# joaospinto/sip_optimal_control

Hardware: AMD Instinct MI355X
Metric: Riccati sweeps/sec (backward+forward) (higher is better)
Workload: dtype f64

## Files before the change

### sip_optimal_control_amd/csrc/chain_qw16.hpp

```cpp
#pragma once
#include <hip/hip_runtime.h>
#include <type_traits>

#include "dpp_blocks_gen.hpp"

namespace sipamd {

template <int I, int E, class F>
__device__ __forceinline__ void sfor(F &&f) {
  if constexpr (I < E) {
    f(std::integral_constant<int, I>{});
    sfor<I + 1, E>(f);
  }
}
template <int I, int E, class F>
__device__ __forceinline__ void sfor_down(F &&f) {
  if constexpr (I > E) {
    f(std::integral_constant<int, I>{});
    sfor_down<I - 1, E>(f);
  }
}

template <int K>
__device__ __forceinline__ double bcast(double x) {
  double und;
  asm volatile("" : "=v"(und));
  return __builtin_amdgcn_update_dpp(und, x, 0x150 + K, 0xf, 0xf, false);
}

__device__ __forceinline__ double rsqrt_nr(double d) {
  const double y = __builtin_amdgcn_rsq(d);
  const double s = d * y;
  const double e = __builtin_fma(-s, y, 1.0);
  const double t = __builtin_fma(0.375, e, 0.5);
  return __builtin_fma(y * e, t, y);
}

__device__ __forceinline__ double rcp_nr(double d) {
  const double y = __builtin_amdgcn_rcp(d);
  const double e = __builtin_fma(-d, y, 1.0);
  const double t = __builtin_fma(e, e, e);
  return __builtin_fma(y, t, y);
}

template <int S>
__device__ __forceinline__ bool chol_ldl_dpp(double (&A)[S], double (&dinv)[S],
                                             const int c) {
#ifdef SIP_QW16_CHOL_SELECT
  unsigned long long failmask = 0;
  sfor<0, S>([&](auto kk) {
    constexpr int k = decltype(kk)::value;
    const double d = bcast<k>(A[k]);
    failmask |= __ballot(d <= 0.0);
    const double y2 = rcp_nr(d);
    dinv[k] = y2;
    const double upd = (c > k && c < S) ? A[k] * y2 : 0.0;
    rank1<S - k - 1, k, true, false>(A + k + 1, A + k + 1, upd);
  });
  return ((failmask >> (__lane_id() & 63)) & 1ull) != 0;
#else
  double dmin = __builtin_inf();
  sfor<0, S>([&](auto kk) {
    constexpr int k = decltype(kk)::value;
    const double d = bcast<k>(A[k]);
    asm("v_min_f64 %0, %1, %2" : "=v"(dmin) : "v"(dmin), "v"(d));
    const double own = A[k] * ((c > k && c < S) ? 1.0 : 0.0);
    const double y2 = rcp_nr(d);
    dinv[k] = y2;
    const double upd = own * y2;
    rank1<S - k - 1, k, true, false>(A + k + 1, A + k + 1, upd);
  });
  return dmin <= 0.0;
#endif
}

template <int S>
__device__ __forceinline__ void ldl_solve_dpp(const double (&Lt)[S],
                                              const double (&dinv)[S],
                                              double (&X)[S]) {
  sfor<0, S>([&](auto jj) {
    constexpr int j = decltype(jj)::value;
    X[j] *= dinv[j];
    rank1<S - j - 1, j, true, (j == 0)>(X + j + 1, Lt + j + 1, X[j]);
  });
  double acc[S];
  sfor<0, S>([&](auto jj) { acc[decltype(jj)::value] = 0.0; });
  sfor_down<S - 1, -1>([&](auto jj) {
    constexpr int j = decltype(jj)::value;
    X[j] = __builtin_fma(-dinv[j], acc[j], X[j]);
    spread<j, false, false>(acc, Lt[j], X[j]);
  });
}

template <int N, int M, bool SYM = false>
struct ChainLayout {
  static constexpr int QLEN = SYM ? N * (N + 1) / 2 : N * N;
  static constexpr int RLEN = SYM ? M * (M + 1) / 2 : M * M;
  static constexpr int NODE = QLEN + N;
  static constexpr int EDGE = N * N + 2 * N * M + RLEN;
  static constexpr int VNODE = 2 * N;
  static constexpr int VEDGE = M;
  static constexpr int GAIN = M * N + M;
  static constexpr int WSN = N * N + 2 * N;
};

template <int N, bool EXPORT = false>
__device__ __forceinline__ bool node_factor(const double (&V)[N], const double dl,
                                            const int c, const double (&E)[N],
                                            const double (&tv)[N], double (&W)[N],
                                            double (&X)[N], double *Lt = nullptr) {
  const double sdi = rsqrt_nr(dl);
  const double sd = dl * sdi;
  double S[N], A[N], rinv[N];
  sfor<0, N>([&](auto ii) { S[decltype(ii)::value] = 0.0; });
  spread<N, false, true>(S, sd, sd);
  sfor<0, N>([&](auto ii) {
    constexpr int r = decltype(ii)::value;
    A[r] = __builtin_fma(S[r], V[r], E[r]);
  });
  const bool fail = chol_ldl_dpp<N>(A, rinv, c);
  if constexpr (EXPORT)
    sfor<0, N>([&](auto ii) { Lt[decltype(ii)::value] = A[decltype(ii)::value]; });
  sfor<0, N>([&](auto ii) { X[decltype(ii)::value] = E[decltype(ii)::value]; });
  spreadv<N, false>(X, sdi, tv);
  ldl_solve_dpp<N>(A, rinv, X);
  sfor<0, N>([&](auto ii) { S[decltype(ii)::value] = 0.0; });
  spread<N, false, true>(S, sdi, sdi);
  sfor<0, N>([&](auto ii) {
    constexpr int r = decltype(ii)::value;
    W[r] = (E[r] - X[r]) * S[r];
  });
  return fail;
}

#ifndef SIP_LQR_NT_SOL
#define SIP_LQR_NT_SOL 0
#endif
#ifndef SIP_LQR_NT_IN
#define SIP_LQR_NT_IN 2
#endif
#ifndef SIP_LQR_NT_FAB
#define SIP_LQR_NT_FAB SIP_LQR_NT_IN
#endif
#ifndef SIP_LQR_NT_FSP
#define SIP_LQR_NT_FSP 0
#endif
typedef __attribute__((address_space(3))) char lds_char;
typedef const __attribute__((address_space(3))) double lds_cdouble;

#ifdef SIP_LQR_STAMPS
#define SIP_STAMP(var)                                                         \
  do {                                                                         \
    __builtin_amdgcn_sched_barrier(0);                                         \
    asm volatile("s_memtime %0\n\ts_waitcnt lgkmcnt(0)" : "=s"(var)::"memory"); \
    __builtin_amdgcn_sched_barrier(0);                                         \
  } while (0)
#define SIP_STAMP_ARG , unsigned long long *__restrict__ stamps
#define SIP_SEG(k)                                                             \
  do {                                                                         \
    unsigned long long now_;                                                   \
    SIP_STAMP(now_);                                                           \
    seg[k] += now_ - seg_last;                                                 \
    seg_last = now_;                                                           \
  } while (0)
#else
#define SIP_SEG(k)                                                             \
  do {                                                                         \
  } while (0)
#define SIP_STAMP(var)                                                         \
  do {                                                                         \
  } while (0)
#define SIP_STAMP_ARG
#endif

template <int PIECES>
struct StageDma {
  static constexpr int INSTR = (4 * PIECES + 63) / 64;
  static constexpr int BYTES = INSTR * 1024;
  static constexpr int ROW_BYTES = PIECES * 16;
#ifdef SIP_QW16_DMA_PLAIN
  static constexpr int GROUP = 1;
#else
  static constexpr int GROUP = 4;
#endif
  static constexpr unsigned BIAS = (GROUP - 1) * 1024u;
  unsigned off[INSTR > 0 ? INSTR : 1];
  __device__ __forceinline__ void init(const int lane,
                                       const unsigned problem_stride_bytes,
                                       const unsigned max_rel) {
    sfor<0, INSTR>([&](auto jj) {
      constexpr int j = decltype(jj)::value;
      const unsigned q = (unsigned)(j * 64 + lane) < 4u * PIECES ? (unsigned)(j * 64 + lane) : 4u * PIECES - 1u;
      unsigned rr = q / PIECES;
      const unsigned within = q - rr * PIECES;
      rr = rr < max_rel ? rr : max_rel;
      off[j] = rr * problem_stride_bytes + within * 16u + BIAS - (unsigned)(j % GROUP) * 1024u;
    });
  }
  template <int AUX = 0>
  __device__ __forceinline__ void issue(const char *base, lds_char *dst,
                                        const int lane) const {
    const char *lowered = base - BIAS;
    sfor<0, INSTR>([&](auto jj) {
      constexpr int j = decltype(jj)::value;
      __builtin_amdgcn_global_load_lds((const __attribute__((address_space(1))) void *)(lowered + off[j]),
                                       (__attribute__((address_space(3))) void *)(dst + (j - j % GROUP) * 1024), 16,
                                       (j % GROUP) * 1024, AUX);
    });
  }
};

template <int DWORDS>
struct StageDmaDwords {
  static constexpr int INSTR = (4 * DWORDS + 63) / 64;
  static constexpr int BYTES = (INSTR * 256 + 1023) / 1024 * 1024;
  static constexpr int ROW_BYTES = DWORDS * 4;
  unsigned off[INSTR > 0 ? INSTR : 1];
  __device__ __forceinline__ void init(const int lane, const unsigned problem_stride_bytes, const unsigned max_rel) {
    sfor<0, INSTR>([&](auto jj) {
      constexpr int j = decltype(jj)::value;
      const unsigned q = (unsigned)(j * 64 + lane) < 4u * DWORDS ? (unsigned)(j * 64 + lane) : 4u * DWORDS - 1u;
      unsigned rr = q / DWORDS;
      const unsigned within = q - rr * DWORDS;
      rr = rr < max_rel ? rr : max_rel;
      off[j] = rr * problem_stride_bytes + within * 4u;
    });
  }
  template <int AUX = 0>
  __device__ __forceinline__ void issue(const char *base, lds_char *dst, const int lane) const {
    sfor<0, INSTR>([&](auto jj) {
      constexpr int j = decltype(jj)::value;
      __builtin_amdgcn_global_load_lds((const __attribute__((address_space(1))) void *)(base + off[j]),
                                       (__attribute__((address_space(3))) void *)(dst + j * 256), 4, 0, AUX);
    });
  }
};

template <int PIECES>
struct StageDmaRows {
  static constexpr int IP = (PIECES + 63) / 64;
  static constexpr int INSTR = 4 * IP;
  static constexpr int ROW_BYTES = IP * 1024;
  static constexpr int BYTES = 4 * ROW_BYTES;
  static constexpr bool RAGGED = PIECES % 64 != 0;
  unsigned vo_main, vo_tail;
  unsigned long long row[4];
  __device__ __forceinline__ void init(const int lane,
                                       const unsigned problem_stride_bytes,
                                       const unsigned max_rel) {
    vo_main = (unsigned)lane * 16u;
    const unsigned last = (unsigned)(PIECES - 1 - 64 * (IP - 1));
    vo_tail = ((unsigned)lane < last ? (unsigned)lane : last) * 16u;
    sfor<0, 4>([&](auto rq) {
      constexpr unsigned r = decltype(rq)::value;
      row[r] = (unsigned long long)(r < max_rel ? r : max_rel) * problem_stride_bytes;
    });
  }
  template <int AUX = 0>
  __device__ __forceinline__ void issue(const char *base, lds_char *dst,
                                        const int lane) const {
    sfor<0, 4>([&](auto rq) {
      constexpr int r = decltype(rq)::value;
      const char *region = base + row[r];
      sfor<0, IP>([&](auto jq) {
        constexpr int jj = decltype(jq)::value;
        constexpr int g = jj / 4;
        const unsigned vo = (RAGGED && jj == IP - 1) ? vo_tail : vo_main;
        __builtin_amdgcn_global_load_lds(
            (const __attribute__((address_space(1))) void *)(region + g * 4096 + vo),
            (__attribute__((address_space(3))) void *)(dst + r * ROW_BYTES + g * 4096), 16, (jj % 4) * 1024, AUX);
      });
    });
  }
};

template <int N, int M, bool WPACK, bool SPLIT = false, bool SYM = false>
struct StagedCfg {
  using L = ChainLayout<N, M, SYM>;
  static_assert(!SYM || (L::QLEN % 2 == 0 && L::RLEN % 2 == 0 && N % 2 == 0 && M % 2 == 0),
                "the symmetric-packed kernels are instantiated where every block stays a whole number of 16-byte pieces");
  static constexpr int AB = N * N + N * M;
  static constexpr int STG = L::NODE + L::EDGE - (SPLIT ? AB : 0);
  static constexpr int WSN =
      WPACK ? ((N * (N + 1) / 2 + 2 * N + 1) / 2) * 2 : L::WSN;
  using BV = StageDma<(L::VNODE + L::VEDGE + 1) / 2>;
  using BMflat = StageDma<(STG + 1) / 2>;
  using BMrows = StageDmaRows<(STG + 1) / 2>;
  struct NoStream {
    static constexpr int INSTR = 0, BYTES = 0, ROW_BYTES = 0;
  };
  static_assert(!SPLIT || AB % 2 == 0, "the split kernels are instantiated for even N (A | B in whole 16-byte pieces)");
  using BA = std::conditional_t<SPLIT, StageDmaRows<AB / 2>, NoStream>;
  static constexpr int SCR_BYTES_ = ((4 * 2 * N + N) * 8 + 1023) / 1024 * 1024;
  static constexpr int waves_per_cu(int bm_bytes) {
    const int per_wave = 2 * (bm_bytes + BA::BYTES + BV::BYTES) + SCR_BYTES_;
    const int w = 163840 / per_wave;
    return w > 4 ? 4 : w;
  }
#ifdef SIP_QW16_DMA_FLAT
  using BM = BMflat;
#else
  using BM = std::conditional_t<SPLIT || waves_per_cu(BMrows::BYTES) >= waves_per_cu(BMflat::BYTES), BMrows, BMflat>;
#endif
  static constexpr int B_BYTES = BM::BYTES + BA::BYTES + BV::BYTES;
  using FA = StageDma<(N * N + N * M + 1) / 2>;
  using FG = std::conditional_t<L::GAIN % 2 == 0, StageDma<L::GAIN / 2>, StageDmaDwords<2 * L::GAIN>>;
  using FW = StageDma<WSN / 2>;
  using FC = std::conditional_t<N % 2 == 0, StageDma<N / 2>, StageDmaDwords<2 * N>>;
  static constexpr int F_BYTES = FA::BYTES + FG::BYTES + FW::BYTES + FC::BYTES;
  static constexpr int F_GLDS = FA::INSTR + FG::INSTR + FW::INSTR + FC::INSTR;
  static constexpr int B_NBUF = 2;
  static constexpr int lds_main(int fbufs) {
    return B_NBUF * B_BYTES > fbufs * F_BYTES ? B_NBUF * B_BYTES : fbufs * F_BYTES;
  }
  static constexpr int waves_with(int fbufs) {
    const int w = 163840 / (lds_main(fbufs) + SCR_BYTES_);
    return w > 4 ? 4 : w;
  }
#ifdef SIP_LQR_FNBUF
  static constexpr int F_NBUF = SIP_LQR_FNBUF;
#else
  static constexpr int F_NBUF = (waves_with(2) > waves_with(3) || lds_main(3) + SCR_BYTES_ > 65536) ? 2 : 3;
#endif
  static constexpr int LDS_MAIN = lds_main(F_NBUF);
  static constexpr int SCR_BYTES = ((4 * 2 * N + N) * 8 + 1023) / 1024 * 1024;
  static constexpr int LDS_BYTES = LDS_MAIN + SCR_BYTES;
  static constexpr bool OK = N <= 16;
  static constexpr bool WIDE = N % 2 == 0;
};

template <int N, int M, bool STAGED, bool WPACK, bool SPLIT = false, bool SYM = false>
__global__ __launch_bounds__(64) void chain_factor_solve_qw16(
    const double *__restrict__ mats, const double *__restrict__ vecs,
    double *__restrict__ sol, double *__restrict__ gains,
    double *__restrict__ wsp, int *__restrict__ status, const long batch,
    const int T, const int mode, double *__restrict__ gfac,
    const double *__restrict__ ab, const long ab_pstride, const long ab_sstride SIP_STAMP_ARG) {
  constexpr bool VDIST = N == 16;
  static_assert(N >= 1 && N <= 16, "one problem per 16-lane row");
  static_assert(M >= 1 && M <= 16, "");
  using L = ChainLayout<N, M, SYM>;
  using C = StagedCfg<N, M, WPACK, SPLIT, SYM>;
  static_assert(!SPLIT || (STAGED && WPACK), "the split kernel is the staged one");
  static_assert(!SYM || (STAGED && !VDIST), "the symmetric-packed layout is served by the staged kernels");
  unsigned long long ts_begin = 0, ts_term = 0, ts_bwd = 0, ts_root = 0,
                     ts_end = 0, ts_a = 0, ts_b = 0, acc_bwait = 0,
                     acc_fwait = 0;
  (void)ts_begin, (void)ts_term, (void)ts_bwd, (void)ts_root, (void)ts_end,
      (void)ts_a, (void)ts_b, (void)acc_bwait, (void)acc_fwait;
  unsigned long long seg[12] = {0, 0, 0, 0, 0, 0, 0, 0, 0, 0, 0, 0}, seg_last = 0;
  (void)seg, (void)seg_last;
  SIP_STAMP(ts_begin);
  static_assert(!STAGED || C::LDS_BYTES <= 65536, "the LDS images of this shape exceed a workgroup's 64 KiB");
  constexpr int STG = C::STG;
  constexpr int OFF_M = L::NODE + (SPLIT ? 0 : N * N + N * M), OFF_R = OFF_M + N * M;
  constexpr int VSTG = L::VNODE + L::VEDGE;
  constexpr int WSN = C::WSN;
  constexpr int WG = WPACK ? N * (N + 1) / 2 : N * N;

  extern __shared__ double lds_raw[];
  lds_char *const lds = (lds_char *)lds_raw;

  const int lane = threadIdx.x & 63;
  const int c = lane & 15;
  const int rr = lane >> 4;
  const long p0 = (long)blockIdx.x * 4;
  long p = p0 + rr;
  const bool valid = p < batch;
  if (!valid)
    p = batch - 1;
  const bool isM = c < N;
  const bool isV = c == N;
  const int cm = isM ? c : N - 1;
  const int cu = c < M ? c : M - 1;

  const long mats_len = (long)(T + 1) * L::NODE + (long)T * (STG - L::NODE);
  const long vecs_len = (long)(T + 1) * L::VNODE + (long)T * L::VEDGE;
  const long gains_len = (long)T * L::GAIN;
  const long ws_len = (long)(T + 1) * WSN;
  const double *pm = mats + p * mats_len;
  const double *pv = vecs + p * vecs_len;
  double *ps = sol + p * vecs_len;
  double *pg = gains + p * gains_len;
  double *pw = wsp + p * ws_len;
  const unsigned max_rel =
      (unsigned)((batch - 1 - p0) < 3 ? (batch - 1 - p0) : 3);

  double E[N];
  sfor<0, N>([&](auto ii) {
    constexpr int r = decltype(ii)::value;
    E[r] = (c == r) ? 1.0 : 0.0;
  });

  auto spill_row_offsets = [&](int(&woff)[N]) {
    sfor<0, N>([&](auto kk) {
      constexpr int k = decltype(kk)::value;
      if constexpr (WPACK) {
        const int lo = k < cm ? k : cm, hi = k < cm ? cm : k;
        woff[k] = lo * N - (lo * (lo - 1)) / 2 + (hi - lo);
      } else {
        woff[k] = cm * N + k;
      }
    });
  };

  int stat = 0;
  double W[N], V[N], t[N], vch[N];
  double vd = 0.0, td = 0.0, qd = 0.0;
  auto sum4 = [](const double (&a)[4]) { return (a[0] + a[1]) + (a[2] + a[3]); };

  const __amdgpu_buffer_rsrc_t ws_rsrc = __builtin_amdgcn_make_buffer_rsrc(
      (void *)(wsp + p0 * ws_len), 0, (int)((max_rel + 1) * ws_len * 8), 0x00020000);
  const int wstore_base = (valid && isM)
                              ? (int)(rr * ws_len * 8) + (c * N - (c * (c - 1)) / 2 - c) * 8
                              : 0x7ffff000;

  typedef __attribute__((address_space(3))) double lds_double;
  lds_char *const scr = lds + C::LDS_MAIN;
  lds_double *const my_t = (lds_double *)(scr + rr * (2 * N * 8));
  lds_double *const my_v = my_t + N;
  lds_cdouble *const zeros = (lds_cdouble *)(scr + 4 * (2 * N * 8));
  if constexpr (STAGED) {
    if (lane < N)
      ((lds_double *)zeros)[lane] = 0.0;
  }

  auto load_vq = [&](auto nm, auto nv, double(&Vq)[N]) {
    if constexpr (SYM) {
      const int base_c = cm * N - (cm * (cm - 1)) / 2 - cm;
      sfor<0, N>([&](auto ii) {
        constexpr int r = decltype(ii)::value;
        constexpr int base_r = r * N - (r * (r - 1)) / 2 - r;
        const int off = r >= cm ? base_c + r : base_r + cm;
        auto src = isV ? nv + r : nm + off;
        Vq[r] = *src;
      });
    } else {
    auto src = isV ? nv : nm + cm * N;
    sfor<0, N>([&](auto ii) {
      constexpr int r = decltype(ii)::value;
      Vq[r] = src[r];
    });
    }
    if constexpr (VDIST)
      qd = nv[cm];
  };

  struct NodeTail {
    double dl, cv[N], dv[N];
    double cd;
  };
  auto load_tail = [&](auto nm, auto nv, NodeTail &nt) {
    const double d = nm[L::QLEN + cm];
    nt.dl = isM ? d : 1.0;
    nt.cd = VDIST ? nv[N + cm] : 0.0;
    if constexpr (std::is_same_v<decltype(nm), lds_cdouble *>) {
      auto csrc = isV ? nv + N : zeros, dsrc = isV ? nm + L::QLEN : zeros;
      sfor<0, N>([&](auto ii) {
        constexpr int r = decltype(ii)::value;
        nt.cv[r] = csrc[r];
        nt.dv[r] = dsrc[r];
      });
    } else {
      sfor<0, N>([&](auto ii) {
        constexpr int r = decltype(ii)::value;
        nt.cv[r] = isV ? nv[N + r] : 0.0;
        nt.dv[r] = isV ? nm[L::QLEN + r] : 0.0;
      });
    }
  };
  auto finish_node = [&](const int i, const NodeTail &nt) {
    const double dl = nt.dl;
    const unsigned long long bad = __ballot(isM && dl <= 0.0);
    const bool bad_row = ((bad >> (lane & 48)) & 0xffffull) != 0;
    if (stat == 0 && bad_row)
      stat = 1;
    double tv[N], X[N];
    sfor<0, N>([&](auto ii) {
      constexpr int r = decltype(ii)::value;
      tv[r] = nt.cv[r] - nt.dv[r] * V[r];
    });
    if constexpr (STAGED && C::WIDE) {
      if (isV) {
        typedef double d2 __attribute__((ext_vector_type(2)));
        typedef __attribute__((address_space(3))) d2 lds_d2;
        lds_d2 *const t2 = (lds_d2 *)my_t, *const v2 = (lds_d2 *)my_v;
        sfor<0, N / 2>([&](auto kk) {
          constexpr int k = decltype(kk)::value;
          t2[k] = d2{tv[2 * k], tv[2 * k + 1]};
          v2[k] = d2{V[2 * k], V[2 * k + 1]};
        });
      }
    } else if constexpr (STAGED) {
      if (isV) {
        sfor<0, N>([&](auto ii) {
          constexpr int r = decltype(ii)::value;
          my_t[r] = tv[r];
          my_v[r] = V[r];
        });
      }
    } else {
      sfor<0, N>([&](auto ii) {
        constexpr int r = decltype(ii)::value;
        t[r] = tv[r];
        vch[r] = V[r];
      });
    }
    if constexpr (VDIST)
      td = nt.cd - dl * vd;
    SIP_SEG(7);
    const bool ffail = node_factor<N>(V, dl, c, E, tv, W, X);
    SIP_SEG(8);
    if (stat == 0 && ffail)
      stat = 2;
    if constexpr (VDIST) {
      const double phi = rsqrt_nr(dl) * td;
      double acc[4] = {0.0, 0.0, 0.0, 0.0};
      dotv<N, true>(acc, phi, X);
      if (valid)
        pw[(long)i * WSN + WG + N + c] = sum4(acc);
    }
    if (valid && isV) {
      double *hn = pw + (long)i * WSN + WG + N;
      sfor<0, N>([&](auto ii) { hn[decltype(ii)::value] = X[decltype(ii)::value]; });
    }
    if constexpr (WPACK) {
      sfor<0, N>([&](auto ii) {
        constexpr int r = decltype(ii)::value;
        const int vo = (r >= c) ? wstore_base : 0x7ffff000;
        typedef unsigned int u32x2 __attribute__((ext_vector_type(2)));
        __builtin_amdgcn_raw_buffer_store_b64(__builtin_bit_cast(u32x2, X[r]), ws_rsrc, vo + r * 8,
                                              i * (WSN * 8), 0);
      });
    } else if (valid && isM) {
      double *wn = pw + (long)i * WSN + c * N;
      sfor<0, N>(
          [&](auto ii) { wn[decltype(ii)::value] = X[decltype(ii)::value]; });
    }
  };

  auto backward_edge = [&](const int i, auto nm, auto ea, auto nv, NodeTail &nt) {

    double F[N], Aaug[N], Bcol[N];
    double Hc[M], G[M], rinvG[M], H[M], K[M];
    {
      auto msrc = isV ? nv + L::VNODE : nm + (OFF_M + cm);
      sfor<0, M>([&](auto jj) {
        constexpr int j = decltype(jj)::value;
        if constexpr (SYM) {
          const int lo = j < cu ? j : cu, hi = j < cu ? cu : j;
          G[j] = nm[OFF_R + lo * M - (lo * (lo - 1)) / 2 + (hi - lo)];
        } else
        G[j] = nm[OFF_R + cu * M + j];
        H[j] = isV ? msrc[j] : msrc[j * N];
      });
    }
    if constexpr (STAGED && C::WIDE) {
      typedef double d2 __attribute__((ext_vector_type(2)));
      typedef const __attribute__((address_space(3))) d2 lds_cd2;
      lds_cd2 *a_src = (lds_cd2 *)(isV ? (lds_cdouble *)my_t : ea + cm * N);
      lds_cd2 *f_src = (lds_cd2 *)(isV ? (lds_cdouble *)my_v : zeros);
      lds_cd2 *b_src = (lds_cd2 *)(ea + N * N + cu * N);
      sfor<0, N / 2>([&](auto kk) {
        constexpr int k = decltype(kk)::value;
        const d2 a2 = a_src[k], f2 = f_src[k], b2 = b_src[k];
        Aaug[2 * k] = a2[0], Aaug[2 * k + 1] = a2[1];
        F[2 * k] = f2[0], F[2 * k + 1] = f2[1];
        Bcol[2 * k] = b2[0], Bcol[2 * k + 1] = b2[1];
      });
    } else if constexpr (STAGED) {
      lds_cdouble *a_src = isV ? (lds_cdouble *)my_t : ea + cm * N;
      lds_cdouble *f_src = isV ? (lds_cdouble *)my_v : zeros;
      lds_cdouble *b_src = ea + N * N + cu * N;
      sfor<0, N>([&](auto kk) {
        constexpr int k = decltype(kk)::value;
        Aaug[k] = a_src[k], F[k] = f_src[k], Bcol[k] = b_src[k];
      });
    } else {
      sfor<0, N>([&](auto kk) {
        constexpr int k = decltype(kk)::value;
        Aaug[k] = isV ? t[k] : ea[cm * N + k];
        F[k] = isV ? vch[k] : 0.0;
        Bcol[k] = ea[N * N + cu * N + k];
      });
    }
    rank1x<N, N, true>(F, W, Aaug);
    if (valid && isV) {
      double *gn = pw + (long)(i + 1) * WSN + WG;
      sfor<0, N>(
          [&](auto ii) { gn[decltype(ii)::value] = F[decltype(ii)::value]; });
    }
    double gd = 0.0, hd = 0.0, hf[M], kf[M];
    if constexpr (VDIST) {
      double acc[4] = {0.0, 0.0, 0.0, 0.0};
      dotv<N, true>(acc, td, W);
      gd = vd + sum4(acc);
      if (valid)
        pw[(long)(i + 1) * WSN + WG + c] = gd;
    }
    SIP_SEG(2);
    asm volatile("" ::: "memory");
    double Vn[N];
    load_vq(nm, nv, Vn);

    sfor<0, M>([&](auto jj) { Hc[decltype(jj)::value] = 0.0; });
    spreadx<M, N, false>(Hc, Bcol, W);
    rank1x<M, N, true>(G, Hc, Bcol);
    SIP_SEG(3);
    const bool gfail = chol_ldl_dpp<M>(G, rinvG, c);
    if (mode == 1 && valid) {
      double *gf = gfac + (p * (long)T + i) * (M * M + M);
      if (c < M)
        sfor<0, M>([&](auto jj) { gf[c * M + decltype(jj)::value] = G[decltype(jj)::value]; });
      if (c == 0)
        sfor<0, M>([&](auto jj) { gf[M * M + decltype(jj)::value] = rinvG[decltype(jj)::value]; });
    }
    SIP_SEG(4);
    if (stat == 0 && gfail)
      stat = 3;

    spreadx<M, N, false>(H, Bcol, F);
    if constexpr (VDIST) {
      double acc[4] = {0.0, 0.0, 0.0, 0.0};
      dotv<N, true>(acc, gd, Bcol);
      hd = nv[L::VNODE + cu] + sum4(acc);
    }
    sfor<0, M>(
        [&](auto jj) { K[decltype(jj)::value] = H[decltype(jj)::value]; });
    ldl_solve_dpp<M>(G, rinvG, K);
    sfor<0, M>(
        [&](auto jj) { K[decltype(jj)::value] = -K[decltype(jj)::value]; });
    if (valid && c <= N) {
      double *gi = pg + (long)i * L::GAIN + c * M;
      sfor<0, M>(
          [&](auto jj) { gi[decltype(jj)::value] = K[decltype(jj)::value]; });
    }
    if constexpr (VDIST) {
      double Lf[M][M];
      sfor<0, M>([&](auto jj) {
        constexpr int j = decltype(jj)::value;
        hf[j] = bcast<j>(hd);
        sfor<0, j>([&](auto iv) {
          constexpr int i2 = decltype(iv)::value;
          Lf[j][i2] = bcast<i2>(G[j]);
        });
      });
      sfor<0, M>([&](auto jj) {
        constexpr int j = decltype(jj)::value;
        double w = hf[j];
        sfor<0, j>([&](auto iv) { w = __builtin_fma(-Lf[j][decltype(iv)::value], kf[decltype(iv)::value], w); });
        kf[j] = w * rinvG[j];
      });
      sfor_down<M - 1, -1>([&](auto jj) {
        constexpr int j = decltype(jj)::value;
        double a = 0.0;
        sfor<j + 1, M>([&](auto iv) { a = __builtin_fma(Lf[decltype(iv)::value][j], kf[decltype(iv)::value], a); });
        kf[j] = __builtin_fma(-rinvG[j], a, kf[j]);
      });
      sfor<0, M>([&](auto jj) { kf[decltype(jj)::value] = -kf[decltype(jj)::value]; });
      if (valid && c == 0) {
        double *gk = pg + (long)i * L::GAIN + N * M;
        sfor<0, M>([&](auto jj) { gk[decltype(jj)::value] = kf[decltype(jj)::value]; });
      }
    }

    SIP_SEG(5);
    spreadx<N, N, false>(Vn, Aaug, F);
    asm volatile("" ::: "memory");
    load_tail(nm, nv, nt);
    asm volatile("" ::: "memory");
    spreadx<N, M, true>(Vn, K, H);
    sfor<0, N>(
        [&](auto ii) { V[decltype(ii)::value] = Vn[decltype(ii)::value]; });
    if constexpr (VDIST) {
      double acc[4] = {0.0, 0.0, 0.0, 0.0};
      dotv<N, true>(acc, gd, Aaug);
      double kh = 0.0;
      sfor<0, M>([&](auto jj) { kh = __builtin_fma(K[decltype(jj)::value], hf[decltype(jj)::value], kh); });
      vd = qd + sum4(acc) + kh;
    }
    SIP_SEG(6);
    asm volatile("" ::: "memory");
  };

  if (mode != 2) {
  typename C::BM dma_bm;
  typename C::BA dma_ba;
  typename C::BV dma_bv;
  auto issue_backward = [&](const int i, lds_char *buf) {
    dma_bm.template issue<SIP_LQR_NT_IN>((const char *)(mats + p0 * mats_len + (long)i * STG), buf, lane);
    if constexpr (SPLIT)
      dma_ba.template issue<SIP_LQR_NT_IN>((const char *)(ab + p0 * ab_pstride + (long)i * ab_sstride),
                                           buf + C::BM::BYTES, lane);
    dma_bv.template issue<SIP_LQR_NT_IN>((const char *)(vecs + p0 * vecs_len + (long)i * VSTG),
                                         buf + C::BM::BYTES + C::BA::BYTES, lane);
  };
  if constexpr (STAGED) {
    dma_bm.init(lane, (unsigned)(mats_len * 8), max_rel);
    if constexpr (SPLIT)
      dma_ba.init(lane, (unsigned)(ab_pstride * 8), max_rel);
    dma_bv.init(lane, (unsigned)(vecs_len * 8), max_rel);
    if (T > 0)
      issue_backward(T - 1, lds + ((T - 1) & 1) * C::B_BYTES);
  }
  {
    NodeTail nt;
    load_vq(pm + (long)T * STG, pv + (long)T * VSTG, V);
    if constexpr (VDIST)
      vd = qd;
    load_tail(pm + (long)T * STG, pv + (long)T * VSTG, nt);
    finish_node(T, nt);
  }
  SIP_STAMP(ts_term);

  auto stage_step = [&](const int i, auto par) {
    SIP_STAMP(ts_a);
#ifdef SIP_LQR_STAMPS
    seg_last = ts_a;
    if (stamps != nullptr && lane == 0 && i < 64)
      stamps[(long)gridDim.x * 24 + (long)blockIdx.x * 128 + i] = ts_a;
#endif
    if constexpr (STAGED) {
      constexpr int PAR = decltype(par)::value;
      lds_char *buf = lds + PAR * C::B_BYTES;
      if constexpr (WPACK)
        asm volatile("s_waitcnt vmcnt(%0)" ::"n"(N) : "memory");
      else
        asm volatile("s_waitcnt vmcnt(0)" ::: "memory");
      SIP_STAMP(ts_b);
      acc_bwait += ts_b - ts_a;
      SIP_SEG(0);
      if (i > 0) {
        issue_backward(i - 1, lds + (PAR ^ 1) * C::B_BYTES);
        asm volatile("" ::: "memory");
      }
      lds_cdouble *nm = (lds_cdouble *)(buf + rr * C::BM::ROW_BYTES);
      lds_cdouble *ea = SPLIT ? (lds_cdouble *)(buf + C::BM::BYTES + rr * C::BA::ROW_BYTES) : nm + L::NODE;
      lds_cdouble *nv = (lds_cdouble *)(buf + C::BM::BYTES + C::BA::BYTES + rr * C::BV::ROW_BYTES);
      SIP_SEG(1);
      NodeTail nt;
      backward_edge(i, nm, ea, nv, nt);
      finish_node(i, nt);
    } else {
      const double *nm = pm + (long)i * STG;
      const double *nv = pv + (long)i * VSTG;
      SIP_SEG(1);
      NodeTail nt;
      backward_edge(i, nm, nm + L::NODE, nv, nt);
      finish_node(i, nt);
    }
    SIP_SEG(9);
  };
#ifdef SIP_QW16_NO_PARITY_UNROLL
  constexpr bool kParityUnroll = false;
#else
  constexpr bool kParityUnroll = STAGED;
#endif
  if constexpr (kParityUnroll) {
    for (int i = (T - 1) | 1; i >= 1; i -= 2) {
      if (i <= T - 1)
        stage_step(i, std::integral_constant<int, 1>{});
      stage_step(i - 1, std::integral_constant<int, 0>{});
    }
  } else if constexpr (STAGED) {
    for (int i = T - 1; i >= 0; --i) {
      if (i & 1)
        stage_step(i, std::integral_constant<int, 1>{});
      else
        stage_step(i, std::integral_constant<int, 0>{});
    }
  } else {
    for (int i = T - 1; i >= 0; --i)
      stage_step(i, std::integral_constant<int, 0>{});
  }

  SIP_STAMP(ts_bwd);
  if constexpr (VDIST) {
    double acc[4] = {0.0, 0.0, 0.0, 0.0};
    dotv<N, true>(acc, td, W);
    if (valid)
      pw[WG + c] = vd + sum4(acc);
  } else {
    double F[N], tt[N];
    sfor<0, N>([&](auto ii) {
      constexpr int r = decltype(ii)::value;
      if constexpr (STAGED) {
        tt[r] = isV ? my_t[r] : 0.0;
        F[r] = isV ? my_v[r] : 0.0;
      } else {
        tt[r] = t[r];
        F[r] = vch[r];
      }
    });
    rank1x<N, N, true>(F, W, tt);
    if (valid && isV) {
      double *gn = pw + WG;
      sfor<0, N>([&](auto ii) { gn[decltype(ii)::value] = F[decltype(ii)::value]; });
    }
  }
  if (valid && c == 0)
    status[p] = stat;
  } else if constexpr (!SPLIT) {
    int woff[N];
    spill_row_offsets(woff);
    auto node_step = [&](const int i, const double v_) {
      const double dl = pm[(long)i * STG + L::QLEN + cm];
      const double t_ = pv[(long)i * VSTG + N + cm] - dl * v_;
      const double sdi = rsqrt_nr(dl);
      const double phi = sdi * t_;
      const double *slot = pw + (long)i * WSN;
      double Srow[N];
      sfor<0, N>([&](auto kk) { Srow[decltype(kk)::value] = slot[woff[decltype(kk)::value]]; });
      double acc[4] = {0.0, 0.0, 0.0, 0.0};
      dotv<N, true>(acc, phi, Srow);
      const double sphi = sum4(acc);
      if (valid && isM)
        pw[(long)i * WSN + WG + N + c] = sphi;
      return sdi * (phi - sphi);
    };
    double v_ = pv[(long)T * VSTG + cm];
    double wt = node_step(T, v_);
    for (int i = T - 1; i >= 0; --i) {
      const double *em = pm + (long)i * STG + L::NODE;
      const double *gi = pg + (long)i * L::GAIN;
      const double *gf = gfac + (p * (long)T + i) * (M * M + M);
      const double gd = v_ + wt;
      if (valid && isM)
        pw[(long)(i + 1) * WSN + WG + c] = gd;
      double Bcol[N], Acol[N], Kc[M], hf[M], kf[M], Lf[M][M], rinv[M];
      sfor<0, N>([&](auto kk) {
        constexpr int k = decltype(kk)::value;
        Bcol[k] = em[N * N + cu * N + k];
        Acol[k] = em[cm * N + k];
      });
      sfor<0, M>([&](auto jj) {
        constexpr int j = decltype(jj)::value;
        Kc[j] = gi[cm * M + j];
        rinv[j] = gf[M * M + j];
        sfor<0, j>([&](auto iv) { Lf[j][decltype(iv)::value] = gf[decltype(iv)::value * M + j]; });
      });
      double acc[4] = {0.0, 0.0, 0.0, 0.0};
      dotv<N, true>(acc, gd, Bcol);
      const double hd = pv[(long)i * VSTG + L::VNODE + cu] + sum4(acc);
      sfor<0, M>([&](auto jj) { hf[decltype(jj)::value] = bcast<decltype(jj)::value>(hd); });
      sfor<0, M>([&](auto jj) {
        constexpr int j = decltype(jj)::value;
        double w = hf[j];
        sfor<0, j>([&](auto iv) { w = __builtin_fma(-Lf[j][decltype(iv)::value], kf[decltype(iv)::value], w); });
        kf[j] = w * rinv[j];
      });
      sfor_down<M - 1, -1>([&](auto jj) {
        constexpr int j = decltype(jj)::value;
        double a = 0.0;
        sfor<j + 1, M>([&](auto iv) { a = __builtin_fma(Lf[decltype(iv)::value][j], kf[decltype(iv)::value], a); });
        kf[j] = __builtin_fma(-rinv[j], a, kf[j]);
      });
      if (valid && c == 0) {
        double *gk = pg + (long)i * L::GAIN + N * M;
        sfor<0, M>([&](auto jj) { gk[decltype(jj)::value] = -kf[decltype(jj)::value]; });
      }
      double acc2[4] = {0.0, 0.0, 0.0, 0.0};
      dotv<N, true>(acc2, gd, Acol);
      double kh = 0.0;
      sfor<0, M>([&](auto jj) { kh = __builtin_fma(Kc[decltype(jj)::value], hf[decltype(jj)::value], kh); });
      v_ = pv[(long)i * VSTG + cm] + sum4(acc2) + kh;
      wt = node_step(i, v_);
    }
    if (valid && isM)
      pw[WG + c] = v_ + wt;
  }

  if (mode == 1)
    return;
  __syncthreads();
  SIP_STAMP(ts_root);


  typename C::FA dma_fa;
  typename C::FG dma_fg;
  typename C::FW dma_fw;
  typename C::FC dma_fd;
  if constexpr (STAGED) {
    dma_fa.init(lane, (unsigned)((SPLIT ? ab_pstride : mats_len) * 8), max_rel);
    dma_fg.init(lane, (unsigned)(gains_len * 8), max_rel);
    dma_fw.init(lane, (unsigned)(ws_len * 8), max_rel);
    dma_fd.init(lane, (unsigned)(mats_len * 8), max_rel);
  }
  auto issue_forward = [&](const int i, lds_char *buf) {
    dma_fa.template issue<SIP_LQR_NT_FAB>(
        (const char *)(SPLIT ? ab + p0 * ab_pstride + (long)i * ab_sstride : mats + p0 * mats_len + (long)i * STG + L::NODE),
        buf, lane);
    dma_fg.template issue<SIP_LQR_NT_FSP>((const char *)(gains + p0 * gains_len + (long)i * L::GAIN),
                 buf + C::FA::BYTES, lane);
    dma_fw.template issue<SIP_LQR_NT_FSP>((const char *)(wsp + p0 * ws_len + (long)(i + 1) * WSN),
                 buf + C::FA::BYTES + C::FG::BYTES, lane);
    dma_fd.template issue<SIP_LQR_NT_FAB>(
        (const char *)(mats + p0 * mats_len + (long)(i + 1) * STG + L::QLEN),
        buf + C::FA::BYTES + C::FG::BYTES + C::FW::BYTES, lane);
  };
  if constexpr (STAGED) {
    if (T > 0)
      issue_forward(0, lds);
    if (C::F_NBUF == 3 && T > 1)
      issue_forward(1, lds + C::F_BYTES);
  }

  double x, y;
  {
    const double gg = pw[WG + cm];
    const double hh = pw[WG + N + cm];
    const double dd = pm[L::QLEN + cm];
    y = gg;
    x = (dd * rsqrt_nr(dd)) * hh;
    if (valid && isM) {
      ps[c] = x;
      ps[N + c] = y;
    }
  }
  int woff[N];
  spill_row_offsets(woff);
  int fbuf = 0;
  for (int i = 0; i < T; ++i) {
    double KT[N], Arow[N], Brow[M], Wc[N];
    double kk0, gg, hh, dd;
    auto read_stage = [&](auto em, auto gi, auto wn, auto dp) {
      sfor<0, N>([&](auto kk) {
        constexpr int k = decltype(kk)::value;
        KT[k] = gi[k * M + cu];
        Arow[k] = em[k * N + cm];
        Wc[k] = wn[woff[k]];
      });
      sfor<0, M>([&](auto jj) {
        constexpr int j = decltype(jj)::value;
        Brow[j] = em[N * N + j * N + cm];
      });
      kk0 = gi[N * M + cu];
      gg = wn[WG + cm];
      hh = wn[WG + N + cm];
      dd = dp[cm];
    };
    SIP_STAMP(ts_a);
#ifdef SIP_LQR_STAMPS
    if (stamps != nullptr && lane == 0 && i < 64)
      stamps[(long)gridDim.x * 24 + (long)blockIdx.x * 128 + 64 + i] = ts_a;
#endif
    if constexpr (STAGED) {
      lds_char *buf = lds + (fbuf * C::F_BYTES);
      static_assert(C::F_GLDS < 64, "vmcnt is 6 bits");
      if (C::F_NBUF == 3 && i + 1 < T)
        asm volatile("s_waitcnt vmcnt(%0)" ::"n"(C::F_GLDS) : "memory");
      else
        asm volatile("s_waitcnt vmcnt(0)" ::: "memory");
      SIP_STAMP(ts_b);
      acc_fwait += ts_b - ts_a;
      lds_char *b1 = buf + C::FA::BYTES, *b2 = b1 + C::FG::BYTES,
               *b3 = b2 + C::FW::BYTES;
      read_stage((lds_cdouble *)(buf + rr * C::FA::ROW_BYTES),
                 (lds_cdouble *)(b1 + rr * C::FG::ROW_BYTES),
                 (lds_cdouble *)(b2 + rr * (WSN * 8)),
                 (lds_cdouble *)(b3 + rr * C::FC::ROW_BYTES));
      asm volatile("s_waitcnt lgkmcnt(0)" ::: "memory");
      if (C::F_NBUF == 2 && i + 1 < T)
        issue_forward(i + 1, lds + (fbuf ^ 1) * C::F_BYTES);
    } else {
      read_stage(pm + (long)i * STG + L::NODE, pg + (long)i * L::GAIN,
                 pw + (long)(i + 1) * WSN, pm + (long)(i + 1) * STG + L::QLEN);
    }

    const double sdi = rsqrt_nr(dd), sdv = dd * sdi;
    double acc[4];
    acc[0] = kk0, acc[1] = 0.0, acc[2] = 0.0, acc[3] = 0.0;
    dotv<N, true>(acc, x, KT);
    const double u = (acc[0] + acc[1]) + (acc[2] + acc[3]);
    acc[0] = 0.0, acc[1] = 0.0, acc[2] = 0.0, acc[3] = 0.0;
    dotv<N, true>(acc, x, Arow);
    dotv<M, true>(acc, u, Brow);
    const double z = (acc[0] + acc[1]) + (acc[2] + acc[3]);
    const double zeta = z * sdi;
    acc[0] = 0.0, acc[1] = 0.0, acc[2] = 0.0, acc[3] = 0.0;
    dotv<N, true>(acc, zeta, Wc);
    const double sz = (acc[0] + acc[1]) + (acc[2] + acc[3]);
    x = sdv * (sz + hh);
    y = __builtin_fma(sdi, zeta - sz, gg);
    if (valid) {
      double *si = ps + (long)i * VSTG;
#if SIP_LQR_NT_SOL
      if (c < M)
        __builtin_nontemporal_store(u, si + 2 * N + c);
      if (isM) {
        __builtin_nontemporal_store(x, si + VSTG + c);
        __builtin_nontemporal_store(y, si + VSTG + N + c);
      }
#else
      if (c < M)
        si[2 * N + c] = u;
      if (isM) {
        si[VSTG + c] = x;
        si[VSTG + N + c] = y;
      }
#endif
    }
    if constexpr (STAGED) {
      asm volatile("" ::: "memory");
      const int nbuf = fbuf >= 1 ? fbuf - 1 : C::F_NBUF - 1;
      if (C::F_NBUF == 3 && i + 2 < T)
        issue_forward(i + 2, lds + nbuf * C::F_BYTES);
      fbuf = fbuf + 1 == C::F_NBUF ? 0 : fbuf + 1;
    }
  }
#ifdef SIP_LQR_STAMPS
  SIP_STAMP(ts_end);
  if (stamps != nullptr && lane == 0) {
    unsigned long long *o = stamps + (long)blockIdx.x * 24;
    o[0] = ts_begin, o[1] = ts_term, o[2] = ts_bwd, o[3] = ts_root;
    o[4] = ts_end, o[5] = acc_bwait, o[6] = acc_fwait;
    o[7] = __builtin_amdgcn_s_memrealtime();
    for (int k = 0; k < 12; ++k)
      o[8 + k] = seg[k];
  }
#endif
}

}
```

Before: 13.28 million.

## Triple-buffer backward-sweep staging and pace DMA issues across compute phases

Adds an optional third LDS buffer for the backward Riccati sweep, so stage i-2 is prefetched while stage i computes. The per-stage global_load_lds instructions are no longer issued as one burst; they are spread over ten pace points inside the edge and node factorisation, using a hand-tuned slot table. The aim is to hide memory latency more deeply and smooth vmcnt pressure. The cost is more LDS per wave, which can reduce occupancy, and the heuristic decides between two and three buffers.

```diff
diff --git a/sip_optimal_control_amd/csrc/chain_qw16.hpp b/sip_optimal_control_amd/csrc/chain_qw16.hpp
--- a/sip_optimal_control_amd/csrc/chain_qw16.hpp
+++ b/sip_optimal_control_amd/csrc/chain_qw16.hpp
@@ -104,11 +104,14 @@
   static constexpr int WSN = N * N + 2 * N;
 };
 
-template <int N, bool EXPORT = false>
+struct NoHook {
+  __device__ __forceinline__ void operator()() const {}
+};
+template <int N, bool EXPORT = false, class Mid = NoHook>
 __device__ __forceinline__ bool node_factor(const double (&V)[N], const double dl,
                                             const int c, const double (&E)[N],
                                             const double (&tv)[N], double (&W)[N],
-                                            double (&X)[N], double *Lt = nullptr) {
+                                            double (&X)[N], double *Lt = nullptr, Mid &&mid = Mid{}) {
   const double sdi = rsqrt_nr(dl);
   const double sd = dl * sdi;
   double S[N], A[N], rinv[N];
@@ -121,6 +124,7 @@
   const bool fail = chol_ldl_dpp<N>(A, rinv, c);
   if constexpr (EXPORT)
     sfor<0, N>([&](auto ii) { Lt[decltype(ii)::value] = A[decltype(ii)::value]; });
+  mid();
   sfor<0, N>([&](auto ii) { X[decltype(ii)::value] = E[decltype(ii)::value]; });
   spreadv<N, false>(X, sdi, tv);
   ldl_solve_dpp<N>(A, rinv, X);
@@ -208,6 +212,13 @@
                                        (j % GROUP) * 1024, AUX);
     });
   }
+  template <int J, int AUX = 0>
+  __device__ __forceinline__ void issue_piece(const char *base, lds_char *dst) const {
+    static_assert(J >= 0 && J < INSTR, "");
+    __builtin_amdgcn_global_load_lds((const __attribute__((address_space(1))) void *)(base - BIAS + off[J]),
+                                     (__attribute__((address_space(3))) void *)(dst + (J - J % GROUP) * 1024), 16,
+                                     (J % GROUP) * 1024, AUX);
+  }
 };
 
 template <int DWORDS>
@@ -233,6 +244,12 @@
       __builtin_amdgcn_global_load_lds((const __attribute__((address_space(1))) void *)(base + off[j]),
                                        (__attribute__((address_space(3))) void *)(dst + j * 256), 4, 0, AUX);
     });
+  }
+  template <int J, int AUX = 0>
+  __device__ __forceinline__ void issue_piece(const char *base, lds_char *dst) const {
+    static_assert(J >= 0 && J < INSTR, "");
+    __builtin_amdgcn_global_load_lds((const __attribute__((address_space(1))) void *)(base + off[J]),
+                                     (__attribute__((address_space(3))) void *)(dst + J * 256), 4, 0, AUX);
   }
 };
 
@@ -272,6 +289,34 @@
       });
     });
   }
+  template <int J, int AUX = 0>
+  __device__ __forceinline__ void issue_piece(const char *base, lds_char *dst) const {
+    static_assert(J >= 0 && J < INSTR, "");
+    constexpr int r = J / IP, jj = J % IP, g = jj / 4;
+    const unsigned vo = (RAGGED && jj == IP - 1) ? vo_tail : vo_main;
+    __builtin_amdgcn_global_load_lds(
+        (const __attribute__((address_space(1))) void *)(base + row[r] + g * 4096 + vo),
+        (__attribute__((address_space(3))) void *)(dst + r * ROW_BYTES + g * 4096), 16, (jj % 4) * 1024, AUX);
+  }
+};
+
+struct PaceSlots {
+  static constexpr int COUNT = 10;
+  static constexpr int of(int k, int pieces) {
+    constexpr int AT[COUNT] = {0, 150, 1350, 1870, 2170, 2630, 3430, 3710, 4710, 5920}, SPAN = 6620;
+#ifdef SIP_LQR_BNOPACE
+    return 0;
+#endif
+    const int due = k * SPAN / pieces;
+    int best = 0;
+    for (int q = 1; q < COUNT; ++q) {
+      const int dq = AT[q] > due ? AT[q] - due : due - AT[q];
+      const int db = AT[best] > due ? AT[best] - due : due - AT[best];
+      if (dq < db)
+        best = q;
+    }
+    return best;
+  }
 };
 
 template <int N, int M, bool WPACK, bool SPLIT = false, bool SYM = false>
@@ -288,6 +333,8 @@
   using BMrows = StageDmaRows<(STG + 1) / 2>;
   struct NoStream {
     static constexpr int INSTR = 0, BYTES = 0, ROW_BYTES = 0;
+    template <int J, int AUX = 0>
+    __device__ __forceinline__ void issue_piece(const char *, lds_char *) const {}
   };
   static_assert(!SPLIT || AB % 2 == 0, "the split kernels are instantiated for even N (A | B in whole 16-byte pieces)");
   using BA = std::conditional_t<SPLIT, StageDmaRows<AB / 2>, NoStream>;
@@ -309,20 +356,27 @@
   using FC = std::conditional_t<N % 2 == 0, StageDma<N / 2>, StageDmaDwords<2 * N>>;
   static constexpr int F_BYTES = FA::BYTES + FG::BYTES + FW::BYTES + FC::BYTES;
   static constexpr int F_GLDS = FA::INSTR + FG::INSTR + FW::INSTR + FC::INSTR;
-  static constexpr int B_NBUF = 2;
-  static constexpr int lds_main(int fbufs) {
-    return B_NBUF * B_BYTES > fbufs * F_BYTES ? B_NBUF * B_BYTES : fbufs * F_BYTES;
-  }
-  static constexpr int waves_with(int fbufs) {
-    const int w = 163840 / (lds_main(fbufs) + SCR_BYTES_);
+  static constexpr int B_GLDS = BM::INSTR + BA::INSTR + BV::INSTR;
+  static constexpr int lds_main(int bbufs, int fbufs) {
+    return bbufs * B_BYTES > fbufs * F_BYTES ? bbufs * B_BYTES : fbufs * F_BYTES;
+  }
+  static constexpr int waves_with(int bbufs, int fbufs) {
+    const int w = 163840 / (lds_main(bbufs, fbufs) + SCR_BYTES_);
     return w > 4 ? 4 : w;
   }
 #ifdef SIP_LQR_FNBUF
   static constexpr int F_NBUF = SIP_LQR_FNBUF;
 #else
-  static constexpr int F_NBUF = (waves_with(2) > waves_with(3) || lds_main(3) + SCR_BYTES_ > 65536) ? 2 : 3;
-#endif
-  static constexpr int LDS_MAIN = lds_main(F_NBUF);
+  static constexpr int F_NBUF = (waves_with(2, 2) > waves_with(2, 3) || lds_main(2, 3) + SCR_BYTES_ > 65536) ? 2 : 3;
+#endif
+#ifdef SIP_LQR_BNBUF
+  static constexpr int B_NBUF = SIP_LQR_BNBUF;
+#else
+  static constexpr int B_NBUF = (waves_with(2, F_NBUF) > waves_with(3, F_NBUF) || lds_main(3, F_NBUF) + SCR_BYTES_ > 65536 ||
+                                 B_GLDS + (WPACK ? N : 0) > 63) ? 2 : 3;
+#endif
+  static_assert(B_NBUF == 2 || B_NBUF == 3, "");
+  static constexpr int LDS_MAIN = lds_main(B_NBUF, F_NBUF);
   static constexpr int SCR_BYTES = ((4 * 2 * N + N) * 8 + 1023) / 1024 * 1024;
   static constexpr int LDS_BYTES = LDS_MAIN + SCR_BYTES;
   static constexpr bool OK = N <= 16;
@@ -469,7 +523,8 @@
       });
     }
   };
-  auto finish_node = [&](const int i, const NodeTail &nt) {
+  auto no_pace = [](auto) {};
+  auto finish_node = [&](const int i, const NodeTail &nt, auto &&pace) {
     const double dl = nt.dl;
     const unsigned long long bad = __ballot(isM && dl <= 0.0);
     const bool bad_row = ((bad >> (lane & 48)) & 0xffffull) != 0;
@@ -509,8 +564,10 @@
     if constexpr (VDIST)
       td = nt.cd - dl * vd;
     SIP_SEG(7);
-    const bool ffail = node_factor<N>(V, dl, c, E, tv, W, X);
+    pace(std::integral_constant<int, 7>{});
+    const bool ffail = node_factor<N>(V, dl, c, E, tv, W, X, nullptr, [&]() { pace(std::integral_constant<int, 8>{}); });
     SIP_SEG(8);
+    pace(std::integral_constant<int, 9>{});
     if (stat == 0 && ffail)
       stat = 2;
     if constexpr (VDIST) {
@@ -539,7 +596,7 @@
     }
   };
 
-  auto backward_edge = [&](const int i, auto nm, auto ea, auto nv, NodeTail &nt) {
+  auto backward_edge = [&](const int i, auto nm, auto ea, auto nv, NodeTail &nt, auto &&pace) {
 
     double F[N], Aaug[N], Bcol[N];
     double Hc[M], G[M], rinvG[M], H[M], K[M];
@@ -600,6 +657,7 @@
     }
     SIP_SEG(2);
     asm volatile("" ::: "memory");
+    pace(std::integral_constant<int, 2>{});
     double Vn[N];
     load_vq(nm, nv, Vn);
 
@@ -607,6 +665,7 @@
     spreadx<M, N, false>(Hc, Bcol, W);
     rank1x<M, N, true>(G, Hc, Bcol);
     SIP_SEG(3);
+    pace(std::integral_constant<int, 3>{});
     const bool gfail = chol_ldl_dpp<M>(G, rinvG, c);
     if (mode == 1 && valid) {
       double *gf = gfac + (p * (long)T + i) * (M * M + M);
@@ -616,6 +675,7 @@
         sfor<0, M>([&](auto jj) { gf[M * M + decltype(jj)::value] = rinvG[decltype(jj)::value]; });
     }
     SIP_SEG(4);
+    pace(std::integral_constant<int, 4>{});
     if (stat == 0 && gfail)
       stat = 3;
 
@@ -665,8 +725,10 @@
     }
 
     SIP_SEG(5);
+    pace(std::integral_constant<int, 5>{});
     spreadx<N, N, false>(Vn, Aaug, F);
     asm volatile("" ::: "memory");
+    pace(std::integral_constant<int, 6>{});
     load_tail(nm, nv, nt);
     asm volatile("" ::: "memory");
     spreadx<N, M, true>(Vn, K, H);
@@ -700,27 +762,76 @@
     if constexpr (SPLIT)
       dma_ba.init(lane, (unsigned)(ab_pstride * 8), max_rel);
     dma_bv.init(lane, (unsigned)(vecs_len * 8), max_rel);
+    if constexpr (C::B_NBUF == 3) {
+      if (T > 0)
+        issue_backward(T - 1, lds + ((T - 1) % 3) * C::B_BYTES);
+      if (T > 1)
+        issue_backward(T - 2, lds + ((T - 2) % 3) * C::B_BYTES);
+    } else {
     if (T > 0)
       issue_backward(T - 1, lds + ((T - 1) & 1) * C::B_BYTES);
-  }
+    }
+  }
+  auto issue_backward_piece = [&](auto kk, const char *src_m, const char *src_a, const char *src_v, lds_char *buf) {
+    constexpr int k = decltype(kk)::value;
+    if constexpr (k < C::BM::INSTR)
+      dma_bm.template issue_piece<k, SIP_LQR_NT_IN>(src_m, buf);
+    else if constexpr (k < C::BM::INSTR + C::BA::INSTR)
+      dma_ba.template issue_piece<k - C::BM::INSTR, SIP_LQR_NT_IN>(src_a, buf + C::BM::BYTES);
+    else
+      dma_bv.template issue_piece<k - C::BM::INSTR - C::BA::INSTR, SIP_LQR_NT_IN>(src_v, buf + C::BM::BYTES + C::BA::BYTES);
+  };
   {
     NodeTail nt;
     load_vq(pm + (long)T * STG, pv + (long)T * VSTG, V);
     if constexpr (VDIST)
       vd = qd;
     load_tail(pm + (long)T * STG, pv + (long)T * VSTG, nt);
-    finish_node(T, nt);
+    finish_node(T, nt, no_pace);
   }
   SIP_STAMP(ts_term);
 
-  auto stage_step = [&](const int i, auto par) {
+  constexpr int kSpillStores = WPACK ? N : 0;
+  auto stage_step = [&](const int i, auto par, auto kind) {
     SIP_STAMP(ts_a);
 #ifdef SIP_LQR_STAMPS
     seg_last = ts_a;
     if (stamps != nullptr && lane == 0 && i < 64)
       stamps[(long)gridDim.x * 24 + (long)blockIdx.x * 128 + i] = ts_a;
 #endif
-    if constexpr (STAGED) {
+    if constexpr (STAGED && C::B_NBUF == 3) {
+      constexpr int PAR = decltype(par)::value;
+      constexpr bool ISSUE = decltype(kind)::value == 0;
+      lds_char *buf = lds + PAR * C::B_BYTES;
+      static_assert(C::B_GLDS + kSpillStores < 64, "vmcnt is 6 bits");
+      asm volatile("s_waitcnt vmcnt(%0)" ::"n"(kSpillStores + (ISSUE ? C::B_GLDS : 0)) : "memory");
+      SIP_STAMP(ts_b);
+      acc_bwait += ts_b - ts_a;
+      SIP_SEG(0);
+      const char *const src_m = (const char *)(mats + p0 * mats_len + (long)(i - 2) * STG);
+      const char *const src_a = SPLIT ? (const char *)(ab + p0 * ab_pstride + (long)(i - 2) * ab_sstride) : nullptr;
+      const char *const src_v = (const char *)(vecs + p0 * vecs_len + (long)(i - 2) * VSTG);
+      lds_char *const nbuf = lds + ((PAR + 1) % 3) * C::B_BYTES;
+      auto pace = [&](auto ss) {
+        if constexpr (ISSUE) {
+          asm volatile("" ::: "memory");
+          sfor<0, C::B_GLDS>([&](auto kk) {
+            if constexpr (PaceSlots::of(decltype(kk)::value, C::B_GLDS) == decltype(ss)::value)
+              issue_backward_piece(kk, src_m, src_a, src_v, nbuf);
+          });
+          asm volatile("" ::: "memory");
+        }
+      };
+      pace(std::integral_constant<int, 0>{});
+      lds_cdouble *nm = (lds_cdouble *)(buf + rr * C::BM::ROW_BYTES);
+      lds_cdouble *ea = SPLIT ? (lds_cdouble *)(buf + C::BM::BYTES + rr * C::BA::ROW_BYTES) : nm + L::NODE;
+      lds_cdouble *nv = (lds_cdouble *)(buf + C::BM::BYTES + C::BA::BYTES + rr * C::BV::ROW_BYTES);
+      SIP_SEG(1);
+      pace(std::integral_constant<int, 1>{});
+      NodeTail nt;
+      backward_edge(i, nm, ea, nv, nt, pace);
+      finish_node(i, nt, pace);
+    } else if constexpr (STAGED) {
       constexpr int PAR = decltype(par)::value;
       lds_char *buf = lds + PAR * C::B_BYTES;
       if constexpr (WPACK)
@@ -739,15 +850,15 @@
       lds_cdouble *nv = (lds_cdouble *)(buf + C::BM::BYTES + C::BA::BYTES + rr * C::BV::ROW_BYTES);
       SIP_SEG(1);
       NodeTail nt;
-      backward_edge(i, nm, ea, nv, nt);
-      finish_node(i, nt);
+      backward_edge(i, nm, ea, nv, nt, no_pace);
+      finish_node(i, nt, no_pace);
     } else {
       const double *nm = pm + (long)i * STG;
       const double *nv = pv + (long)i * VSTG;
       SIP_SEG(1);
       NodeTail nt;
-      backward_edge(i, nm, nm + L::NODE, nv, nt);
-      finish_node(i, nt);
+      backward_edge(i, nm, nm + L::NODE, nv, nt, no_pace);
+      finish_node(i, nt, no_pace);
     }
     SIP_SEG(9);
   };
@@ -756,22 +867,47 @@
 #else
   constexpr bool kParityUnroll = STAGED;
 #endif
-  if constexpr (kParityUnroll) {
+  constexpr std::integral_constant<int, 0> c0{};
+  constexpr std::integral_constant<int, 1> c1{};
+  constexpr std::integral_constant<int, 2> c2{};
+  if constexpr (STAGED && C::B_NBUF == 3) {
+    if (T >= 3) {
+      int skip = (4 - (T - 1) % 3) % 3;
+      for (int i = T - 1 + skip; i >= 4; i -= 3) {
+        switch (skip) {
+        case 0:
+          stage_step(i, c1, c0);
+          [[fallthrough]];
+        case 1:
+          stage_step(i - 1, c0, c0);
+          [[fallthrough]];
+        default:
+          stage_step(i - 2, c2, c0);
+        }
+        skip = 0;
+      }
+    }
+    if (T >= 2)
+      stage_step(1, c1, c1);
+    if (T >= 1)
+      stage_step(0, c0, c1);
+    asm volatile("s_waitcnt vmcnt(0)" ::: "memory");
+  } else if constexpr (kParityUnroll) {
     for (int i = (T - 1) | 1; i >= 1; i -= 2) {
       if (i <= T - 1)
-        stage_step(i, std::integral_constant<int, 1>{});
-      stage_step(i - 1, std::integral_constant<int, 0>{});
+        stage_step(i, c1, c0);
+      stage_step(i - 1, c0, c0);
     }
   } else if constexpr (STAGED) {
     for (int i = T - 1; i >= 0; --i) {
       if (i & 1)
-        stage_step(i, std::integral_constant<int, 1>{});
+        stage_step(i, c1, c0);
       else
-        stage_step(i, std::integral_constant<int, 0>{});
+        stage_step(i, c0, c0);
     }
   } else {
     for (int i = T - 1; i >= 0; --i)
-      stage_step(i, std::integral_constant<int, 0>{});
+      stage_step(i, c0, c0);
   }
 
   SIP_STAMP(ts_bwd);
```

After: 12.91 million. 0.972x the previous value.
